# gregbugaj/marie-icr

Measured on AMD Instinct MI355X. Metric: pages/sec (2550x3300, ~40 lines/page), higher is better.
Workload: dtype f16; 1 GPU; BASELINE configs[2]: full detect->crop->recognize, 64 synthetic 2550x3300x3 u8 pages per GPU per step resident in HBM; DiT-base Mask R-CNN detector (resize to 1035x800, 1 pass, 8 pages per forward) + TrOCR-base recognizer on the generator's 40 ground-truth line boxes per page (fixed work), beam 3, 15+1 decoder steps; seeded random weights; f16 operands with fp32 accumulation is the 16-bit mode of ; crops_per_page=40

## Files before the change

include/marie_hip.h:

```cpp
#ifndef MARIE_HIP_H
#define MARIE_HIP_H

#include <stddef.h>
#include <stdint.h>

#ifdef __cplusplus
extern "C" {
#endif

#define MHIP_OK 0
#define MHIP_EINVAL (-22)
#define MHIP_ENOMEM (-12)
#define MHIP_EHIP (-5)
#define MHIP_ESTATE (-1)

#define MHIP_PREC_F16 0
#define MHIP_PREC_F32 1

typedef struct mhip_ctx mhip_ctx;
typedef struct mhip_crnn mhip_crnn;

int mhip_init(int device_id, mhip_ctx** out);
int mhip_destroy(mhip_ctx* ctx);
const char* mhip_last_error(mhip_ctx* ctx);
// ... 236 lines not shown
  int max_positions;
  int beam;
  int max_len_b;
  int min_len;
  int pad, eos;
  float embed_scale;
  int img_size;
} mhip_trocr_config;
int mhip_trocr_default_config(int model , mhip_trocr_config* cfg);
int mhip_trocr_max_len(const mhip_trocr_config* cfg);
int mhip_trocr_create(mhip_ctx* ctx, int precision, const mhip_trocr_config* cfg, mhip_trocr** out);
int mhip_trocr_destroy(mhip_trocr* m);
int mhip_trocr_set_tensor(mhip_trocr* m, const char* key, const float* data, const int64_t* shape, int ndim);
int mhip_trocr_finalize(mhip_trocr* m);
int mhip_trocr_alloc_arena(mhip_trocr* m);
int mhip_trocr_arena(mhip_trocr* m, int which , void** arena_dev, size_t* bytes);
size_t mhip_trocr_workspace_bytes(mhip_trocr* m, int n);
int mhip_trocr_set_decode_gate(mhip_trocr* m, mhip_gate* gate);
int mhip_trocr_generate(mhip_trocr* m, const uint8_t* crops_dev, int n, int swap_rb, int32_t* tokens_out,
                        int32_t* lengths_out, float* scores_out);
int mhip_trocr_generate_host(mhip_trocr* m, const uint8_t* crops_host, int n, int swap_rb, int32_t* tokens_out,
                             int32_t* lengths_out, float* scores_out, float* enc_tokens_out, float* step0_logits_out);
int mhip_trocr_encode_begin(mhip_trocr* m, int max_crops);
int mhip_trocr_encode_fragments(mhip_trocr* m, const uint8_t* base_dev, const mhip_crop_desc* descs_host, int n, int swap_rb);
int mhip_trocr_encoded(mhip_trocr* m);
int mhip_trocr_decode(mhip_trocr* m, int32_t* tokens_out, int32_t* lengths_out, float* scores_out);
int mhip_trocr_generate_fragments(mhip_trocr* m, const uint8_t* base_dev, const mhip_crop_desc* descs_host, int n,
                                  int swap_rb, int32_t* tokens_out, int32_t* lengths_out, float* scores_out);
int mhip_trocr_generate_trace_host(mhip_trocr* m, const uint8_t* crops_host, int n, int swap_rb, int32_t* tokens_out,
                                   int32_t* lengths_out, float* scores_out, float* trace_scores, int32_t* trace_tokens,
                                   int32_t* trace_beams, int* steps_out);
int mhip_cross_attention_host(mhip_ctx* ctx, const float* q, const float* enc, const float* wk, const float* wv,
                              const float* bv, int crops, int beam, int heads, int n_tok, int enc_dim, float* out);
int mhip_decode_attention_host(mhip_ctx* ctx, int precision, int heads, int n_keys, int nq, int rows, int slots, int kv_rows,
                               const float* q, const float* k, const float* v, const int32_t* anc, int anc_ld,
                               int force_generic, float* out);

typedef struct mhip_layoutlmv3 mhip_layoutlmv3;
typedef struct mhip_layoutlmv3_config {
  int hidden, layers, heads, ffn;
  int vocab, type_vocab;
  int max_position_embeddings;
  int max_2d_position_embeddings;
  int coordinate_size, shape_size;
  int input_size, patch;
  int rel_pos_bins, max_rel_pos;
  int rel_2d_pos_bins, max_rel_2d_pos;
  float layer_norm_eps;
  int pad_id;
  int num_labels;
  int max_text;
} mhip_layoutlmv3_config;
int mhip_layoutlmv3_default_config(mhip_layoutlmv3_config* cfg);
int mhip_layoutlmv3_create(mhip_ctx* ctx, int precision, const mhip_layoutlmv3_config* cfg, mhip_layoutlmv3** out);
int mhip_layoutlmv3_destroy(mhip_layoutlmv3* m);
int mhip_layoutlmv3_set_tensor(mhip_layoutlmv3* m, const char* key, const float* data, const int64_t* shape, int ndim);
int mhip_layoutlmv3_finalize(mhip_layoutlmv3* m);
int mhip_layoutlmv3_alloc_arena(mhip_layoutlmv3* m);
int mhip_layoutlmv3_arena(mhip_layoutlmv3* m, void** arena_dev, size_t* bytes);
int mhip_layoutlmv3_set_resample(mhip_layoutlmv3* m, int filter);
int mhip_layoutlmv3_seq_len(const mhip_layoutlmv3_config* cfg);
int mhip_layoutlmv3_bucket(int relative_position, int num_buckets, int max_distance);
int mhip_layoutlmv3_classify(mhip_layoutlmv3* m, const uint8_t* base_dev, const mhip_crop_desc* pages_host, int n,
                             const int32_t* ids, const int32_t* bbox, const int32_t* attention_mask, float* logits_out);
int mhip_layoutlmv3_hidden_host(mhip_layoutlmv3* m, const uint8_t* pages_host, size_t pages_bytes,
                                const mhip_crop_desc* pages_desc, int n, const int32_t* ids, const int32_t* bbox,
// ... 65 lines not shown
```

marie_icr_amd/_lib.py:

```python
from __future__ import annotations

import ctypes as C
import os
import weakref

import numpy as np

_HERE = os.path.dirname(os.path.abspath(__file__))
LIB_PATH = os.environ.get("MARIE_HIP_LIB") or os.path.join(_HERE, "libmarie_hip.so")

PREC_F16 = 0
PREC_F32 = 1

_vp, _i, _sz = C.c_void_p, C.c_int, C.c_size_t
_SIGNATURES = (
    ("mhip_init", _i, [_i, C.POINTER(_vp)]),
    ("mhip_destroy", _i, [_vp]),
    ("mhip_last_error", C.c_char_p, [_vp]),
    ("mhip_set_stream", _i, [_vp, _vp]),
    ("mhip_synchronize", _i, [_vp]),
    ("mhip_device_info", _i, [_vp, C.c_char_p, _sz, C.POINTER(_i), C.POINTER(_sz)]),
    ("mhip_memcpy_dev", _i, [_vp, _vp, _vp, _sz]),
    ("mhip_gate_create", _i, [_vp, C.POINTER(_vp)]),
    ("mhip_gate_destroy", _i, [_vp]),
# ... 64 lines not shown
    ("mhip_det_final_multi_host", _i, [_vp, _vp, _i, _vp, _i, _i, _i, _i, _i, _i, C.c_float, C.c_float, _i, _vp, _vp,
                                       _vp, _vp]),
    ("mhip_register_warp", _i, [_vp, _vp, _i, _i, C.c_size_t, _vp, _vp, _vp]),
    ("mhip_register_warp_host", _i, [_vp, _vp, _i, _i, _vp, _vp]),
    ("mhip_blackout_bboxes", _i, [_vp, _vp, _i, _i, _vp, _i, C.POINTER(_i)]),
    ("mhip_content_extents", _i, [_vp, _vp, _i, _i, _vp, _i, _i, _vp]),
    ("mhip_overlay_create", _i, [_vp, _i, _i, C.POINTER(_vp)]),
    ("mhip_overlay_destroy", _i, [_vp]),
    ("mhip_overlay_set_tensor", _i, [_vp, C.c_char_p, _vp, C.POINTER(C.c_int64), _i]),
    ("mhip_overlay_finalize", _i, [_vp]),
    ("mhip_overlay_padded_shape", _i, [_i, _i, C.POINTER(_i), C.POINTER(_i)]),
    ("mhip_overlay_forward", _i, [_vp, _vp, _i, _i, _vp]),
    ("mhip_overlay_forward_host", _i, [_vp, _vp, _i, _i, _vp, _vp]),
    ("mhip_overlay_blend", _i, [_vp, _vp, _vp, _vp, _sz]),
    ("mhip_trocr_default_config", _i, [_i, _vp]),
    ("mhip_trocr_max_len", _i, [_vp]),
    ("mhip_trocr_create", _i, [_vp, _i, _vp, C.POINTER(_vp)]),
    ("mhip_trocr_destroy", _i, [_vp]),
    ("mhip_trocr_set_tensor", _i, [_vp, C.c_char_p, _vp, C.POINTER(C.c_int64), _i]),
    ("mhip_trocr_finalize", _i, [_vp]),
    ("mhip_trocr_alloc_arena", _i, [_vp]),
    ("mhip_trocr_arena", _i, [_vp, _i, C.POINTER(_vp), C.POINTER(_sz)]),
    ("mhip_trocr_workspace_bytes", _sz, [_vp, _i]),
    ("mhip_trocr_set_decode_gate", _i, [_vp, _vp]),
    ("mhip_trocr_generate", _i, [_vp, _vp, _i, _i, _vp, _vp, _vp]),
    ("mhip_trocr_generate_host", _i, [_vp, _vp, _i, _i, _vp, _vp, _vp, _vp, _vp]),
    ("mhip_trocr_generate_fragments", _i, [_vp, _vp, _vp, _i, _i, _vp, _vp, _vp]),
    ("mhip_trocr_encode_begin", _i, [_vp, _i]),
    ("mhip_trocr_encode_fragments", _i, [_vp, _vp, _vp, _i, _i]),
    ("mhip_trocr_encoded", _i, [_vp]),
    ("mhip_trocr_decode", _i, [_vp, _vp, _vp, _vp]),
    ("mhip_trocr_generate_trace_host", _i, [_vp, _vp, _i, _i, _vp, _vp, _vp, _vp, _vp, _vp, C.POINTER(_i)]),
    ("mhip_cross_attention_host", _i, [_vp, _vp, _vp, _vp, _vp, _vp, _i, _i, _i, _i, _i, _vp]),
    ("mhip_decode_attention_host", _i, [_vp, _i, _i, _i, _i, _i, _i, _i, _vp, _vp, _vp, _vp, _i, _i, _vp]),
    ("mhip_gemm_ln_fold", _i, [_vp, _i, _vp]),
    ("mhip_ln_finalize", _i, [_vp, _vp, _i, _i, _vp, _vp, _i, _i, C.c_float]),
    ("mhip_token_init_split", _i, [_vp, _vp, _vp, _vp, _vp, _vp, _i, _i, _i, _i, _i]),
    ("mhip_layoutlmv3_default_config", _i, [_vp]),
    ("mhip_layoutlmv3_create", _i, [_vp, _i, _vp, C.POINTER(_vp)]),
    ("mhip_layoutlmv3_destroy", _i, [_vp]),
    ("mhip_layoutlmv3_set_tensor", _i, [_vp, C.c_char_p, _vp, C.POINTER(C.c_int64), _i]),
    ("mhip_layoutlmv3_finalize", _i, [_vp]),
    ("mhip_layoutlmv3_alloc_arena", _i, [_vp]),
    ("mhip_layoutlmv3_arena", _i, [_vp, C.POINTER(_vp), C.POINTER(_sz)]),
    ("mhip_layoutlmv3_set_resample", _i, [_vp, _i]),
    ("mhip_layoutlmv3_seq_len", _i, [_vp]),
    ("mhip_layoutlmv3_bucket", _i, [_i, _i, _i]),
    ("mhip_layoutlmv3_max_token_labels", _i, [_i]),
    ("mhip_layoutlmv3_classify", _i, [_vp, _vp, _vp, _i, _vp, _vp, _vp, _vp]),
    ("mhip_layoutlmv3_hidden_host", _i, [_vp, _vp, _sz, _vp, _i, _vp, _vp, _vp, _vp, _vp, _vp]),
    ("mhip_layoutlmv3_tag", _i, [_vp, _vp, _vp, _i, _vp, _i, _vp, _vp, _vp, _vp, _vp, _vp]),
    ("mhip_layoutlmv3_tag_host", _i, [_vp, _vp, _sz, _vp, _i, _vp, _i, _vp, _vp, _vp, _vp, _vp, _vp]),
    ("mhip_token_head_host", _i, [_vp, _i, _i, _i, _i, _vp, _vp, _vp, _vp, _vp, _vp, _vp, _vp]),
    ("mhip_attention_bias_host", _i, [_vp, _i, _i, _i, _vp, _vp, _vp, _vp, _vp, _vp, _vp, _vp, _vp, _vp, _i, _i, _i, _i, _vp]),
    ("mhip_vq_template_create", _i, [_vp, _vp, _i, _i, _i, _vp, _vp, _i, C.POINTER(_vp)]),
    ("mhip_vq_template_destroy", _i, [_vp]),
    ("mhip_vq_template_state", _i, [_vp, C.POINTER(_i), C.POINTER(_i), _vp, _vp]),
    ("mhip_vq_template_set_filters", _i, [_vp, _vp, _vp]),
    ("mhip_vq_match", _i, [_vp, _vp, _i, _i, _sz, _vp, _i, _i, _i, _vp, _i, _i, _vp]),
    ("mhip_vq_assign_host", _i, [_vp, _vp, _i, _i, _vp, _vp, _i, _vp]),
    ("mhip_vq_kmeans_step_host", _i, [_vp, _vp, _i, _i, _vp, _vp, _i, _vp, _vp, _vp, C.POINTER(C.c_double)]),
    ("mhip_vq_heatmap_host", _i, [_vp, _vp, _i, _i, _i, _vp, _vp, _vp, _vp]),
    ("mhip_vq_peaks_host", _i, [_vp, _vp, _i, _i, _i, _vp, _i, _vp]),
    ("mhip_clip_cosine_host", _i, [_vp, _vp, _vp, _i, _i, _i, _vp]),
    ("mhip_max_page_size", _i, [_i, _i, _i, _i, C.c_double, C.POINTER(_i), C.POINTER(_i)]),
    ("mhip_resize_area_u8", _i, [_vp, _vp, _i, _i, _i, C.c_size_t, _vp, _i, _i]),
# ... 296 lines not shown
```

marie_icr_amd/csrc/common.h:

```cpp
#pragma once
#include <hip/hip_runtime.h>
#include <stdint.h>
#include <stdio.h>
#include <string.h>

#include <mutex>
#include <string>
#include <vector>

#include "../../include/marie_hip.h"

enum MhipKernelId {
  MHIP_K_CONV_FIRST = 0,
  MHIP_K_CONV_IGEMM = 1,
  MHIP_K_LSTM_REC = 2,
  MHIP_K_CTC_DECODE = 3,
  MHIP_K_IMAGE_OPS = 4,
  MHIP_K_CCL = 5,
  MHIP_K_CROP_BATCH = 6,
  MHIP_K_ATTN = 7,
  MHIP_K_ATTN_FLASH = 8,
  MHIP_K_VIT_OPS = 9,
  MHIP_K_DET_OPS = 10,
  MHIP_K_DEC_OPS = 11,
// ... 299 lines not shown
int mhip_launch_subsample2(mhip_ctx* ctx, int precision, const void* in, void* out, int B, int H, int W, int C);

int mhip_launch_layernorm2(mhip_ctx* ctx, int precision, const float* x, const float* g, const float* b, float* y_f32,
                           void* y_t, int rows, int D, float eps);
int mhip_launch_embed_step(mhip_ctx* ctx, int precision, const int* tokens, const void* emb, const float* pos_row, float scale,
                           const float* g, const float* b, float* x, void* xt, int rows, int D, float eps);
constexpr int DEC_ATTN_MAX_KEYS = 640;
struct DecAttnDesc {
  const void* q = nullptr;
  const void* k = nullptr;
  const void* v = nullptr;
  void* out = nullptr;
  const int* anc = nullptr;
  int anc_ld = 0, slots = 0;
  int kv_rows = 0;
  int ldq = 0, ldk = 0, ldo = 0;
  int heads = 0, groups = 0, nq = 1, n_keys = 0;
  int force_generic = 0;
};
int mhip_launch_decode_attention(mhip_ctx* ctx, int precision, const DecAttnDesc& d);
struct CrossAbsorbDesc {
  const void* q = nullptr;
  int ldq = 0;
  const void* E = nullptr;
  int kv_rows = 0, n_keys = 0, enc_dim = 0;
  const void* wkt = nullptr;
  const void* wv = nullptr;
  const float* bv = nullptr;
  void* qt = nullptr;
  void* ct = nullptr;
  void* ao = nullptr;
  int ldo = 0;
  int crops = 0, beam = 1, heads = 0;
};
bool mhip_cross_absorb_supported(int enc_dim, int beam, int heads);
int mhip_launch_cross_absorbed(mhip_ctx* ctx, const CrossAbsorbDesc& d);
struct BeamCandDesc {
  const void* logits = nullptr;
  int logits_f16 = 0;
  int ld = 0, vocab = 0, beam = 1, bsz = 0;
  const float* cum = nullptr;
  int step = 0, max_len = 0, min_len = 1, pad = 1, eos = 2;
  float* cand_scores = nullptr;
  int* cand_tokens = nullptr;
  int* cand_beams = nullptr;
};
int mhip_launch_beam_candidates(mhip_ctx* ctx, const BeamCandDesc& d);
int mhip_launch_ancestry(mhip_ctx* ctx, const int* anc_old, int* anc_new, const int* parent, int rows, int ld, int step);
struct BeamState {
  int bsz = 0, beam = 1, max_len = 0, pad = 1, eos = 2;
  const float* cand_scores = nullptr;
  const int* cand_tokens = nullptr;
  const int* cand_beams = nullptr;
  int* tokens[2] = {nullptr, nullptr};
  int* last_tok = nullptr;
  int* parent = nullptr;
  float* cum = nullptr;
  unsigned char* ignore = nullptr;
  unsigned char* finished = nullptr;
  int* fin_count = nullptr;
  int* fin_tokens = nullptr;
  int* fin_len = nullptr;
  float* fin_score = nullptr;
  int* remaining = nullptr;
};
void mhip_beam_state_carve(Carver& ws, int bsz, int beam, int max_len, int pad, int eos, BeamState* st);
// ... 48 lines not shown
```

marie_icr_amd/csrc/cross_attn.hip:

```cpp
#include <math.h>

#include "common.h"

namespace {

typedef _Float16 half8v __attribute__((ext_vector_type(8)));
typedef _Float16 half4v __attribute__((ext_vector_type(4)));
typedef __fp16 fp16x4 __attribute__((__vector_size__(4 * sizeof(__fp16))));
typedef float float4v __attribute__((ext_vector_type(4)));

#ifndef CA_E_AUX
#define CA_E_AUX 2
#endif
__device__ __forceinline__ void glds16(const void* gsrc, void* lds_wave_base) {
  __builtin_amdgcn_global_load_lds((const __attribute__((address_space(1))) void*)gsrc,
                                   (__attribute__((address_space(3))) void*)lds_wave_base, 16, 0, CA_E_AUX);
}
__device__ __forceinline__ half4v lds_tr16(const char* p) {
  fp16x4 v = __builtin_amdgcn_ds_read_tr16_b64_v4f16((__attribute__((address_space(3))) fp16x4*)p);
  return __builtin_bit_cast(half4v, v);
}
__device__ __forceinline__ int swz(int row) { return ((row & 7) << 1) | ((row >> 3) & 1); }

template <int N>
__device__ __forceinline__ void wait_vm() {
  asm volatile("s_waitcnt vmcnt(%0)" ::"n"(N) : "memory");
}
template <int PER, int MAXT>
__device__ __forceinline__ void wait_vm_dyn(int tiles) {
  if constexpr (MAXT <= 0 || PER <= 0) {
    wait_vm<0>();
  } else {
    if (tiles >= MAXT) wait_vm<PER * MAXT>();
    else wait_vm_dyn<PER, MAXT - 1>(tiles);
  }
}

struct CrossArgs {
  const _Float16* E;
  const _Float16* qt;
  _Float16* ct;
  size_t crop_stride, tile_stride;
  int n_keys, heads;
};

#ifndef CA_TK
#define CA_TK 32
#endif
constexpr int TK = CA_TK;
static_assert(TK == 16 || TK == 32, "cross_attn key tile");
constexpr int RT = TK / 16;
constexpr int cross_slots(int ed, int w) {
  const int n = (160 * 1024 - 4 * w * 1024) / (TK * ed * 2);
  return n > 6 ? 6 : n;
}

template <int ED, int W, int NPW, int NI, bool FEED>
__device__ __forceinline__ void cross_tile(const char* __restrict__ sb, char* __restrict__ feed_dst, float4v* __restrict__ xb,
                                           const char* __restrict__ feed_src, const int (&dma_off)[NPW],
                                           const int (&a_off)[4], const int (&t_off)[8], const half8v (&qf)[ED / 64],
                                           float4v (&acc)[ED / 32], float& mref, float& lsum, int t, int n_keys, int wave, int lane) {
  constexpr int NW = 2 * W, ROWB = ED * 2, KS = ED / 64, MT = ED / 32;
  const int g = lane >> 4;
#ifdef CA_DMA_ONLY
    if (FEED) {
#pragma unroll
      for (int j = 0; j < NPW; ++j) {
        const int i = wave + j * NW;
        if (NI % NW == 0 || i < NI) glds16(feed_src + dma_off[j], feed_dst + i * 1024);
      }
    }
    if (CA_DMA_ONLY) __builtin_amdgcn_s_barrier();
    return;
#endif
    float4v s[2] = {(float4v){0.f, 0.f, 0.f, 0.f}, (float4v){0.f, 0.f, 0.f, 0.f}};
    constexpr int EVERY = (KS / NPW) > 0 ? (KS / NPW) : 1;
    constexpr int AHEAD = KS < 4 ? KS : 4;
    half8v a0[KS], a1[RT == 2 ? KS : 1];
#pragma unroll
    for (int ks = 0; ks < AHEAD; ++ks) {
      a0[ks] = *(const half8v*)(sb + a_off[ks & 3] + 256 * (ks >> 2));
      if (RT == 2) a1[ks] = *(const half8v*)(sb + a_off[ks & 3] + 256 * (ks >> 2) + 16 * ROWB);
    }
    __builtin_amdgcn_sched_barrier(0);
#pragma unroll
    for (int ks = 0; ks < KS; ++ks) {
      if (ks + AHEAD < KS) {
        a0[ks + AHEAD] = *(const half8v*)(sb + a_off[(ks + AHEAD) & 3] + 256 * ((ks + AHEAD) >> 2));
        if (RT == 2) a1[ks + AHEAD] = *(const half8v*)(sb + a_off[(ks + AHEAD) & 3] + 256 * ((ks + AHEAD) >> 2) + 16 * ROWB);
      }
      if (FEED && ks % EVERY == 0 && ks / EVERY < NPW) {
        const int j = ks / EVERY, i = wave + j * NW;
        if (NI % NW == 0 || i < NI) glds16(feed_src + dma_off[j], feed_dst + i * 1024);
      }
      __builtin_amdgcn_sched_barrier(0);
      s[0] = __builtin_amdgcn_mfma_f32_16x16x32_f16(a0[ks], qf[ks], s[0], 0, 0, 0);
      if (RT == 2) s[1] = __builtin_amdgcn_mfma_f32_16x16x32_f16(a1[RT == 2 ? ks : 0], qf[ks], s[1], 0, 0, 0);
      __builtin_amdgcn_sched_barrier(0);
    }
    if (FEED) {
#pragma unroll
      for (int j = (KS + EVERY - 1) / EVERY; j < NPW; ++j) {
        const int i = wave + j * NW;
        if (NI % NW == 0 || i < NI) glds16(feed_src + dma_off[j], feed_dst + i * 1024);
      }
    }
    xb[(wave * 2 + 0) * 64 + lane] = s[0];
    if (RT == 2) xb[(wave * 2 + 1) * 64 + lane] = s[1];
    __builtin_amdgcn_s_waitcnt(0xc07f);
    __builtin_amdgcn_s_barrier();
    s[0] += xb[((wave ^ 1) * 2 + 0) * 64 + lane];
    if (RT == 2) s[1] += xb[((wave ^ 1) * 2 + 1) * 64 + lane];
    const int key0 = t * TK;
    if (key0 + TK > n_keys) {
#pragma unroll
      for (int mt = 0; mt < RT; ++mt)
#pragma unroll
        for (int e = 0; e < 4; ++e)
          if (key0 + 16 * mt + 4 * g + e >= n_keys) s[mt][e] = -INFINITY;
    }
    float mx = fmaxf(fmaxf(s[0][0], s[0][1]), fmaxf(s[0][2], s[0][3]));
    if (RT == 2) mx = fmaxf(mx, fmaxf(fmaxf(s[1][0], s[1][1]), fmaxf(s[1][2], s[1][3])));
    mx = fmaxf(mx, __shfl_xor(mx, 16));
    mx = fmaxf(mx, __shfl_xor(mx, 32));
    if (t == 0) {
      mref = mx;
    } else if (__builtin_amdgcn_ballot_w64(mx > mref + 8.f) != 0) {
      const float nr = fmaxf(mref, mx), f = __builtin_amdgcn_exp2f(mref - nr);
      mref = nr;
      lsum *= f;
#pragma unroll
      for (int i = 0; i < MT; ++i) acc[i] *= f;
    }
    half8v pf = (half8v){0, 0, 0, 0, 0, 0, 0, 0};
#pragma unroll
    for (int mt = 0; mt < RT; ++mt)
#pragma unroll
      for (int e = 0; e < 4; ++e) {
// ... 12 lines not shown
    __builtin_amdgcn_sched_barrier(0);
#pragma unroll
    for (int mt = 0; mt < MT; ++mt) {
      if (mt + TAHEAD < MT) {
        tlo[mt + TAHEAD] = lds_tr16(sb + t_off[(mt + TAHEAD) & 7] + 256 * ((mt + TAHEAD) >> 3));
        if (RT == 2) thi[mt + TAHEAD] = lds_tr16(sb + t_off[(mt + TAHEAD) & 7] + 256 * ((mt + TAHEAD) >> 3) + 16 * ROWB);
      }
      __builtin_amdgcn_sched_barrier(0);
      if constexpr (RT == 2) {
        const half8v a = __builtin_shufflevector(tlo[mt], thi[mt], 0, 1, 2, 3, 4, 5, 6, 7);
        acc[mt] = __builtin_amdgcn_mfma_f32_16x16x32_f16(a, pf, acc[mt], 0, 0, 0);
      } else {
        acc[mt] = __builtin_amdgcn_mfma_f32_16x16x16f16(tlo[mt], pf4, acc[mt], 0, 0, 0);
      }
      __builtin_amdgcn_sched_barrier(0);
    }
}

template <int ED, int W>
__global__ __launch_bounds__(128 * W) void cross_attn_kernel(CrossArgs p) {
  extern __shared__ __attribute__((aligned(16))) char smem[];
  constexpr int NW = 2 * W;
  constexpr int ROWB = ED * 2;
  constexpr int HB = ED;
  constexpr int TILE_B = TK * ROWB;
  constexpr int NS = cross_slots(ED, W);
  constexpr int NI = TILE_B / 1024;
  constexpr int NPW = (NI + NW - 1) / NW;
  constexpr int KS = ED / 64, MT = ED / 32;
  const int tid = threadIdx.x, lane = tid & 63;
  const int wave = __builtin_amdgcn_readfirstlane(tid >> 6);
  const int beam = wave >> 1, hh = wave & 1;
  const int n = lane & 15, g = lane >> 4;
  const int crop = blockIdx.x;
  const char* Ec = (const char*)p.E + (size_t)crop * p.crop_stride;
  const int ntiles = (p.n_keys + TK - 1) / TK;
  float4v* xbuf = (float4v*)(smem + NS * TILE_B);

  int dma_off[NPW];
#pragma unroll
  for (int j = 0; j < NPW; ++j) {
    const int i = wave + j * NW;
    const int byte = i * 1024 + lane * 16;
    const int r = byte / ROWB, cp = (byte - r * ROWB) >> 4;
    const int c = (cp & ~15) | ((cp & 15) ^ swz(r));
    dma_off[j] = r * ROWB + c * 16;
  }
  auto issue = [&](int t, int slot) {
    const char* src = Ec + (size_t)t * p.tile_stride;
    char* dst = smem + slot * TILE_B;
#pragma unroll
    for (int j = 0; j < NPW; ++j) {
      const int i = wave + j * NW;
      if (NI % NW == 0 || i < NI) glds16(src + dma_off[j], dst + i * 1024);
    }
  };
  const bool short_wave = (NI % NW != 0) && (wave + (NPW - 1) * NW >= NI);

  half8v qf[KS];
  {
    const _Float16* qr = p.qt + ((size_t)(crop * W + beam) * 16 + n) * ED + hh * (ED / 2) + g * 8;
#pragma unroll
    for (int ks = 0; ks < KS; ++ks) {
      if (n < p.heads) qf[ks] = *(const half8v*)(qr + ks * 32);
      else qf[ks] = (half8v){0, 0, 0, 0, 0, 0, 0, 0};
    }
  }
  int a_off[4];
#pragma unroll
  for (int j = 0; j < 4; ++j) a_off[j] = n * ROWB + hh * HB + 16 * ((4 * j + g) ^ swz(n));
  int t_off[8];
  {
    const int q = n >> 2, pp = n & 3, row = 4 * g + q, x = swz(row);
#pragma unroll
    for (int j = 0; j < 8; ++j) t_off[j] = row * ROWB + hh * HB + 32 * (j ^ (x >> 1)) + 16 * ((pp >> 1) ^ (x & 1)) + 8 * (pp & 1);
  }

  float4v acc[MT];
#pragma unroll
  for (int i = 0; i < MT; ++i) acc[i] = (float4v){0.f, 0.f, 0.f, 0.f};
  float mref = 0.f, lsum = 0.f;

  constexpr int DEPTH = NS - 1;
  static_assert(NS >= 2 && DEPTH * NPW <= 60, "ring depth / vmcnt range");
#pragma unroll
  for (int i = 0; i < DEPTH; ++i)
    if (i < ntiles) issue(i, i);
  int slot = 0;
  const int nfeed = ntiles > DEPTH ? ntiles - DEPTH : 0;
  for (int t = 0; t < nfeed; ++t) {
    if (short_wave) wait_vm<(NPW - 1) * (DEPTH - 1)>();
    else wait_vm<NPW * (DEPTH - 1)>();
    __builtin_amdgcn_s_barrier();
    const char* feed_src = Ec + (size_t)(t + DEPTH) * p.tile_stride;
    char* feed_dst = smem + (slot == 0 ? NS - 1 : slot - 1) * TILE_B;
    cross_tile<ED, W, NPW, NI, true>(smem + slot * TILE_B, feed_dst, xbuf, feed_src, dma_off, a_off, t_off, qf, acc, mref, lsum, t,
                                     p.n_keys, wave, lane);
    slot = (slot == NS - 1) ? 0 : slot + 1;
  }
  for (int t = nfeed; t < ntiles; ++t) {
    const int after = min(DEPTH - 1, ntiles - 1 - t);
    if (short_wave) wait_vm_dyn<NPW - 1, DEPTH - 1>(after);
    else wait_vm_dyn<NPW, DEPTH - 1>(after);
    __builtin_amdgcn_s_barrier();
    cross_tile<ED, W, NPW, NI, false>(smem + slot * TILE_B, smem, xbuf, Ec, dma_off, a_off, t_off, qf, acc, mref, lsum, t, p.n_keys,
                                      wave, lane);
    slot = (slot == NS - 1) ? 0 : slot + 1;
  }
  lsum += __shfl_xor(lsum, 16);
  lsum += __shfl_xor(lsum, 32);
  const float inv = 1.f / lsum;
  if (n < p.heads) {
    _Float16* o = p.ct + ((size_t)(crop * W + beam) * 16 + n) * ED + hh * (ED / 2) + 4 * g;
#pragma unroll
    for (int mt = 0; mt < MT; ++mt) {
      half4v h;
#pragma unroll
      for (int e = 0; e < 4; ++e) h[e] = (_Float16)(acc[mt][e] * inv);
      *(half4v*)(o + 16 * mt) = h;
    }
  }
}

template <int ED>
__global__ __launch_bounds__(256) void absorb_q_kernel(const _Float16* __restrict__ q, int ldq, const _Float16* __restrict__ wkt,
                                                      _Float16* __restrict__ qt, int rows) {
  __shared__ __attribute__((aligned(16))) _Float16 stage[4][64][72];
  const int lane = threadIdx.x & 63, wave = threadIdx.x >> 6, n = lane & 15, g = lane >> 4;
  const int h = blockIdx.y, r0 = blockIdx.x * 64;
  half8v b[4][2];
#pragma unroll
  for (int nt = 0; nt < 4; ++nt)
#pragma unroll
    for (int ks = 0; ks < 2; ++ks) {
      const int r = r0 + nt * 16 + n;
      if (r < rows) b[nt][ks] = *(const half8v*)(q + (size_t)r * ldq + h * 64 + ks * 32 + g * 8);
      else b[nt][ks] = (half8v){0, 0, 0, 0, 0, 0, 0, 0};
    }
  constexpr int MTW = ED / 64;
  const _Float16* wrow = wkt + ((size_t)h * ED + wave * (ED / 4) + n) * 64 + g * 8;
#pragma unroll 1
  for (int mg = 0; mg < MTW / 4; ++mg) {
#pragma unroll
    for (int mi = 0; mi < 4; ++mi) {
      const int mt = mg * 4 + mi;
      const half8v a0 = *(const half8v*)(wrow + (size_t)mt * 16 * 64);
      const half8v a1 = *(const half8v*)(wrow + (size_t)mt * 16 * 64 + 32);
#pragma unroll
      for (int nt = 0; nt < 4; ++nt) {
        float4v c = {0.f, 0.f, 0.f, 0.f};
        c = __builtin_amdgcn_mfma_f32_16x16x32_f16(a0, b[nt][0], c, 0, 0, 0);
        c = __builtin_amdgcn_mfma_f32_16x16x32_f16(a1, b[nt][1], c, 0, 0, 0);
        half4v o;
// ... 36 lines not shown
    for (int mt = 0; mt < 4; ++mt) a[mt] = *(const half8v*)(arow + (size_t)mt * 16 * ED + ks * 32);
#pragma unroll
    for (int mt = 0; mt < 4; ++mt)
#pragma unroll
      for (int nt = 0; nt < 4; ++nt) c[mt][nt] = __builtin_amdgcn_mfma_f32_16x16x32_f16(a[mt], b[nt], c[mt][nt], 0, 0, 0);
  }
#pragma unroll
  for (int mt = 0; mt < 4; ++mt)
#pragma unroll
    for (int nt = 0; nt < 4; ++nt) part[wave][mt * 4 + nt][lane] = c[mt][nt];
  __syncthreads();
  const int r = r0 + wave * 16 + n;
#pragma unroll
  for (int mt = 0; mt < 4; ++mt) {
    float4v v = part[0][mt * 4 + wave][lane];
#pragma unroll
    for (int w = 1; w < 4; ++w) v += part[w][mt * 4 + wave][lane];
    const float4v bb = *(const float4v*)(bv + h * 64 + mt * 16 + 4 * g);
    half4v o;
#pragma unroll
    for (int e = 0; e < 4; ++e) o[e] = (_Float16)(v[e] + bb[e]);
    if (r < rows) *(half4v*)(ao + (size_t)r * ldo + h * 64 + mt * 16 + 4 * g) = o;
  }
}

template <int ED>
int launch_ed(mhip_ctx* ctx, const CrossAbsorbDesc& d) {
  const int rows = d.crops * d.beam;
  PROF_LAUNCH(ctx, MHIP_K_DEC_OPS, hipLaunchKernelGGL((absorb_q_kernel<ED>), dim3((rows + 63) / 64, d.heads), dim3(256), 0, ctx->stream,
                                                     (const _Float16*)d.q, d.ldq, (const _Float16*)d.wkt, (_Float16*)d.qt, rows));
  CrossArgs a;
  a.E = (const _Float16*)d.E; a.qt = (const _Float16*)d.qt; a.ct = (_Float16*)d.ct;
  constexpr int TILE_B = TK * ED * 2;
  a.n_keys = d.n_keys; a.heads = d.heads;
  a.crop_stride = (size_t)d.kv_rows * ED * 2; a.tile_stride = TILE_B;
  const size_t lds = (size_t)cross_slots(ED, d.beam) * TILE_B + (size_t)d.beam * 4096;
#define CROSS_LAUNCH(WV)                                                                                                       \
  do {                                                                                                                         \
    static std::once_flag attr;                                                                                                \
    std::call_once(attr, [&] {                                                                                                 \
      (void)hipFuncSetAttribute((const void*)cross_attn_kernel<ED, WV>, hipFuncAttributeMaxDynamicSharedMemorySize, (int)lds); \
    });                                                                                                                        \
    PROF_LAUNCH(ctx, MHIP_K_CROSS_ATTN,                                                                                        \
                hipLaunchKernelGGL((cross_attn_kernel<ED, WV>), dim3(d.crops), dim3(128 * WV), lds, ctx->stream, a));          \
  } while (0)
  switch (d.beam) {
    case 1: CROSS_LAUNCH(1); break;
    case 2: CROSS_LAUNCH(2); break;
    case 3: CROSS_LAUNCH(3); break;
    default: CROSS_LAUNCH(4); break;
  }
#undef CROSS_LAUNCH
  PROF_LAUNCH(ctx, MHIP_K_DEC_OPS, hipLaunchKernelGGL((absorb_v_kernel<ED>), dim3((rows + 63) / 64, d.heads), dim3(256), 0, ctx->stream,
                                                     (const _Float16*)d.ct, (const _Float16*)d.wv, d.bv, (_Float16*)d.ao, d.ldo, rows));
  hipError_t e = hipGetLastError();
  if (e != hipSuccess) return mhip_fail(ctx, MHIP_EHIP, "cross_attn launch: %s", hipGetErrorString(e));
  return 0;
}

}

bool mhip_cross_absorb_supported(int enc_dim, int beam, int heads) {
  return (enc_dim == 256 || enc_dim == 512 || enc_dim == 768 || enc_dim == 1024) && beam >= 1 && beam <= 4 && heads >= 1 && heads <= 16;
}

int mhip_launch_cross_absorbed(mhip_ctx* ctx, const CrossAbsorbDesc& d) {
  if (!d.q || !d.E || !d.wkt || !d.wv || !d.bv || !d.qt || !d.ct || !d.ao || d.crops < 1)
    return mhip_fail(ctx, MHIP_EINVAL, "cross_attn: null operand");
  if (!mhip_cross_absorb_supported(d.enc_dim, d.beam, d.heads) || d.n_keys < 1 || d.kv_rows < d.n_keys || d.ldq % 8 || d.ldo % 4)
    return mhip_fail(ctx, MHIP_EINVAL, "cross_attn: unsupported shape (enc_dim %d, beam %d, heads %d)", d.enc_dim, d.beam, d.heads);
  switch (d.enc_dim) {
    case 256: return launch_ed<256>(ctx, d);
    case 512: return launch_ed<512>(ctx, d);
    case 768: return launch_ed<768>(ctx, d);
    default: return launch_ed<1024>(ctx, d);
  }
}
// ... 1 lines not shown
```

marie_icr_amd/csrc/trocr_api.hip:

```cpp
#include <math.h>

#include "vit_internal.h"

struct mhip_trocr {
  mhip_ctx* ctx = nullptr;
  int precision = MHIP_PREC_F16;
  mhip_trocr_config cfg{};
  mhip_vit* vit = nullptr;
  TensorStore store;
  Arena arena;
  bool ready = false;
  uint8_t* frag_crops = nullptr;
  size_t frag_crops_bytes = 0;
  void* frag_scratch = nullptr;
  size_t frag_scratch_bytes = 0;
  bool absorb = false;
  mhip_gate* decode_gate = nullptr;
  int* h_remaining = nullptr;
  hipEvent_t rem_ev[2] = {nullptr, nullptr};
  char* enc_store = nullptr;
  int enc_cap = 0, enc_count = 0;
  size_t esz() const { return precision == MHIP_PREC_F16 ? 2 : 4; }
};

// ... 545 lines not shown
      MHIP_HIP(ctx, hipMalloc(&m->frag_scratch, scratch));
      m->frag_scratch_bytes = scratch;
    }
  }
  VitRun run;
  run.tokens_dst = m->enc_store + (size_t)m->enc_count * vg.npad * c.enc_dim * es;
  int rc = mhip_carve_workspace(ctx, [&](Carver& ws) { vit_carve(m->vit, ws, n, vg, &run); });
  if (rc) return rc;
  rc = mhip_pil_resize_fragments(ctx, base_dev, descs_host, n, m->frag_crops, S, S, MHIP_PIL_BICUBIC, m->frag_scratch, m->frag_scratch_bytes);
  if (rc) return rc;
  if ((rc = vit_encode(m->vit, m->frag_crops, n, S, S, S, S, swap_rb, &run))) return rc;
  m->enc_count += n;
  return MHIP_OK;
}

extern "C" int mhip_trocr_decode(mhip_trocr* m, int32_t* tokens_out, int32_t* lengths_out, float* scores_out) {
  if (!m || !tokens_out || !lengths_out || !scores_out) return MHIP_EINVAL;
  mhip_ctx* ctx = m->ctx;
  if (m->enc_count < 1) return mhip_fail(ctx, MHIP_EINVAL, "trocr: nothing encoded since mhip_trocr_encode_begin");
  MHIP_HIP(ctx, hipSetDevice(ctx->device));
  const int n = m->enc_count;
  VitGeom vg;
  vit_geometry(m->vit, m->cfg.img_size, m->cfg.img_size, &vg);
  TrocrDecodeBufs b;
  int rc = mhip_carve_workspace(ctx, [&](Carver& ws) { trocr_decode_carve(m, ws, n, vg, false, &b); });
  if (rc) return rc;
  MHIP_HIP(ctx, hipMemsetAsync(m->enc_store + (size_t)n * vg.npad * m->cfg.enc_dim * m->esz(), 0, (size_t)64 * m->cfg.enc_dim * m->esz(), ctx->stream));
  rc = trocr_decode(m, b, m->enc_store, vg, n, tokens_out, lengths_out, scores_out, nullptr, nullptr);
  m->enc_count = 0;
  return rc;
}


extern "C" int mhip_cross_attention_host(mhip_ctx* ctx, const float* q, const float* enc, const float* wk, const float* wv,
                                         const float* bv, int crops, int beam, int heads, int n_tok, int enc_dim, float* out) {
  if (!ctx || !q || !enc || !wk || !wv || !bv || !out || crops < 1 || n_tok < 1) return MHIP_EINVAL;
  if (!mhip_cross_absorb_supported(enc_dim, beam, heads)) return mhip_fail(ctx, MHIP_EINVAL, "cross_attention: unsupported shape");
  MHIP_HIP(ctx, hipSetDevice(ctx->device));
  const int D = heads * 64, M = crops * beam, npad = (n_tok + 7) / 8 * 8;
  const size_t rowsE = (size_t)crops * npad + 64;
  std::vector<_Float16> hq((size_t)M * D), hE(rowsE * enc_dim, (_Float16)0.f), hkt((size_t)D * enc_dim), hwv((size_t)D * enc_dim);
  for (size_t i = 0; i < hq.size(); ++i) hq[i] = (_Float16)q[i];
  for (int c = 0; c < crops; ++c)
    for (int s = 0; s < n_tok; ++s)
      for (int d = 0; d < enc_dim; ++d) hE[((size_t)c * npad + s) * enc_dim + d] = (_Float16)enc[((size_t)c * n_tok + s) * enc_dim + d];
  const float log2e = 1.4426950408889634f;
  for (int h = 0; h < heads; ++h)
    for (int d = 0; d < enc_dim; ++d)
      for (int j = 0; j < 64; ++j) hkt[((size_t)h * enc_dim + d) * 64 + j] = (_Float16)(wk[(size_t)(h * 64 + j) * enc_dim + d] * log2e);
  for (size_t i = 0; i < hwv.size(); ++i) hwv[i] = (_Float16)wv[i];
  const size_t scr = (size_t)M * 16 * enc_dim * 2;
  char *dq = nullptr, *dE = nullptr, *dkt = nullptr, *dwv = nullptr, *qt = nullptr, *ct = nullptr, *ao = nullptr;
  float* dbv = nullptr;
  int rc = mhip_carve_workspace(ctx, [&](Carver& ws) {
    dq = ws.take(hq.size() * 2); dE = ws.take(hE.size() * 2); dkt = ws.take(hkt.size() * 2);
    dwv = ws.take(hwv.size() * 2); dbv = ws.take<float>((size_t)D * 4);
    qt = ws.take(scr); ct = ws.take(scr); ao = ws.take((size_t)M * D * 2);
  });
  if (rc) return rc;
  MHIP_HIP(ctx, hipMemcpyAsync(dq, hq.data(), hq.size() * 2, hipMemcpyHostToDevice, ctx->stream));
  MHIP_HIP(ctx, hipMemcpyAsync(dE, hE.data(), hE.size() * 2, hipMemcpyHostToDevice, ctx->stream));
  MHIP_HIP(ctx, hipMemcpyAsync(dkt, hkt.data(), hkt.size() * 2, hipMemcpyHostToDevice, ctx->stream));
  MHIP_HIP(ctx, hipMemcpyAsync(dwv, hwv.data(), hwv.size() * 2, hipMemcpyHostToDevice, ctx->stream));
  MHIP_HIP(ctx, hipMemcpyAsync(dbv, bv, (size_t)D * 4, hipMemcpyHostToDevice, ctx->stream));
  CrossAbsorbDesc cd;
  cd.q = dq; cd.ldq = D; cd.E = dE; cd.kv_rows = npad; cd.n_keys = n_tok; cd.enc_dim = enc_dim;
  cd.wkt = dkt; cd.wv = dwv; cd.bv = dbv; cd.qt = qt; cd.ct = ct; cd.ao = ao; cd.ldo = D;
  cd.crops = crops; cd.beam = beam; cd.heads = heads;
  if ((rc = mhip_launch_cross_absorbed(ctx, cd))) return rc;
  std::vector<_Float16> ho((size_t)M * D);
  MHIP_HIP(ctx, hipMemcpyAsync(ho.data(), ao, ho.size() * 2, hipMemcpyDeviceToHost, ctx->stream));
  MHIP_HIP(ctx, hipStreamSynchronize(ctx->stream));
  for (size_t i = 0; i < ho.size(); ++i) out[i] = (float)ho[i];
  return MHIP_OK;
}

template <typename T>
static void to_elems(const float* src, size_t n, std::vector<char>& dst, size_t off, size_t count, size_t src_ld, size_t dst_ld) {
  T* d = (T*)dst.data();
  for (size_t i = 0; i < count; ++i)
    for (size_t j = 0; j < n; ++j) d[off + i * dst_ld + j] = (T)src[i * src_ld + j];
}

extern "C" int mhip_decode_attention_host(mhip_ctx* ctx, int precision, int heads, int n_keys, int nq, int rows, int slots,
                                          int kv_rows, const float* q, const float* k, const float* v, const int32_t* anc,
                                          int anc_ld, int force_generic, float* out) {
  if (!ctx || !q || !k || !v || !out) return MHIP_EINVAL;
  if (precision != MHIP_PREC_F16 && precision != MHIP_PREC_F32) return mhip_fail(ctx, MHIP_EINVAL, "unknown precision %d", precision);
  if (heads < 1 || heads > 16 || n_keys < 1 || nq < 1 || rows < 1 || rows % nq)
    return mhip_fail(ctx, MHIP_EINVAL, "decode_attention_host: heads %d n_keys %d nq %d rows %d", heads, n_keys, nq, rows);
  const bool self = anc != nullptr;
  if (self && (nq != 1 || slots < 1 || anc_ld < std::min(n_keys, DEC_ATTN_MAX_KEYS + 1)))
    return mhip_fail(ctx, MHIP_EINVAL, "decode_attention_host: self-attention needs nq 1, slots >= 1, anc_ld >= n_keys");
  if (!self && kv_rows < n_keys) return mhip_fail(ctx, MHIP_EINVAL, "decode_attention_host: kv_rows %d < n_keys %d", kv_rows, n_keys);
  const int hist = std::min(n_keys, DEC_ATTN_MAX_KEYS + 1);
  if (self)
    for (int r = 0; r < rows; ++r)
      for (int s = 0; s < hist; ++s)
        if (anc[(size_t)r * anc_ld + s] < 0 || anc[(size_t)r * anc_ld + s] >= slots)
          return mhip_fail(ctx, MHIP_EINVAL, "decode_attention_host: ancestry slot out of range at row %d step %d", r, s);
  MHIP_HIP(ctx, hipSetDevice(ctx->device));
  const int D = heads * 64, groups = rows / nq;
  const size_t es = precision == MHIP_PREC_F16 ? 2 : 4;
  const int ldq = self ? 3 * D : D, ldk = self ? 3 * D : D;
  const size_t nq_el = (size_t)rows * ldq;
  const size_t nk_el = self ? (size_t)hist * slots * ldk : (size_t)groups * kv_rows * D;
  std::vector<char> hq(nq_el * es), hk(nk_el * es), hv(self ? 0 : nk_el * es);
// ... 47 lines not shown
```

Before: 95.89 pages/s.

## Make cross-attention kernel persistent across crops with continuous tile prefetch

The cross-attention kernel now launches at most one block per CU, and each block loops over several crops. Its DMA ring keeps prefetching tiles straight from one crop into the next, and it also prefetches the next crop's query fragments, so the pipeline never drains between crops. The last tile of each crop fetches only the rows it needs instead of the padded tile, and the ring is zeroed when that path matters. Vmcnt is now tracked dynamically, which adds bookkeeping and branchy waitcnt selection. A test entry point exposes the grid cap and the padding value.

Result: no change. 95.69 pages/s (median of 2 runs) (-0.2%).

```diff
diff --git a/include/marie_hip.h b/include/marie_hip.h
--- a/include/marie_hip.h
+++ b/include/marie_hip.h
@@ -292,6 +292,9 @@
                                    int32_t* trace_beams, int* steps_out);
 int mhip_cross_attention_host(mhip_ctx* ctx, const float* q, const float* enc, const float* wk, const float* wv,
                               const float* bv, int crops, int beam, int heads, int n_tok, int enc_dim, float* out);
+int mhip_cross_attention_host_ex(mhip_ctx* ctx, const float* q, const float* enc, const float* wk, const float* wv,
+                                 const float* bv, int crops, int beam, int heads, int n_tok, int enc_dim, int grid_cap,
+                                 float pad_value, float* out);
 int mhip_decode_attention_host(mhip_ctx* ctx, int precision, int heads, int n_keys, int nq, int rows, int slots, int kv_rows,
                                const float* q, const float* k, const float* v, const int32_t* anc, int anc_ld,
                                int force_generic, float* out);
diff --git a/marie_icr_amd/_lib.py b/marie_icr_amd/_lib.py
--- a/marie_icr_amd/_lib.py
+++ b/marie_icr_amd/_lib.py
@@ -120,6 +120,7 @@
     ("mhip_trocr_decode", _i, [_vp, _vp, _vp, _vp]),
     ("mhip_trocr_generate_trace_host", _i, [_vp, _vp, _i, _i, _vp, _vp, _vp, _vp, _vp, _vp, C.POINTER(_i)]),
     ("mhip_cross_attention_host", _i, [_vp, _vp, _vp, _vp, _vp, _vp, _i, _i, _i, _i, _i, _vp]),
+    ("mhip_cross_attention_host_ex", _i, [_vp, _vp, _vp, _vp, _vp, _vp, _i, _i, _i, _i, _i, _i, C.c_float, _vp]),
     ("mhip_decode_attention_host", _i, [_vp, _i, _i, _i, _i, _i, _i, _i, _vp, _vp, _vp, _vp, _i, _i, _vp]),
     ("mhip_gemm_ln_fold", _i, [_vp, _i, _vp]),
     ("mhip_ln_finalize", _i, [_vp, _vp, _i, _i, _vp, _vp, _i, _i, C.c_float]),
diff --git a/marie_icr_amd/csrc/common.h b/marie_icr_amd/csrc/common.h
--- a/marie_icr_amd/csrc/common.h
+++ b/marie_icr_amd/csrc/common.h
@@ -355,6 +355,7 @@
   void* ao = nullptr;
   int ldo = 0;
   int crops = 0, beam = 1, heads = 0;
+  int grid_cap = 0;
 };
 bool mhip_cross_absorb_supported(int enc_dim, int beam, int heads);
 int mhip_launch_cross_absorbed(mhip_ctx* ctx, const CrossAbsorbDesc& d);
diff --git a/marie_icr_amd/csrc/cross_attn.hip b/marie_icr_amd/csrc/cross_attn.hip
--- a/marie_icr_amd/csrc/cross_attn.hip
+++ b/marie_icr_amd/csrc/cross_attn.hip
@@ -36,12 +36,39 @@
   }
 }
 
+template <int LO, int HI>
+__device__ __forceinline__ void wait_vm_range(int n) {
+  if constexpr (LO == HI) {
+    wait_vm<LO>();
+  } else {
+    constexpr int MID = (LO + HI + 1) / 2;
+    if (n >= MID) wait_vm_range<MID, HI>(n);
+    else wait_vm_range<LO, MID - 1>(n);
+  }
+}
+template <int OFF>
+__device__ __forceinline__ void load_q16(half8v& d, const _Float16* p) {
+  asm volatile("global_load_dwordx4 %0, %1, off offset:%2" : "=&v"(d) : "v"(p), "n"(OFF) : "memory");
+}
+template <int KS, int I = 0>
+__device__ __forceinline__ void load_q(half8v (&qf)[KS], const _Float16* p) {
+  if constexpr (I < KS) {
+    load_q16<I * 64>(qf[I], p);
+    load_q<KS, I + 1>(qf, p);
+  }
+}
+template <int KS>
+__device__ __forceinline__ void pin_q(half8v (&qf)[KS]) {
+#pragma unroll
+  for (int ks = 0; ks < KS; ++ks) asm volatile("" : "+v"(qf[ks]));
+}
+
 struct CrossArgs {
   const _Float16* E;
   const _Float16* qt;
   _Float16* ct;
   size_t crop_stride, tile_stride;
-  int n_keys, heads;
+  int n_keys, heads, crops;
 };
 
 #ifndef CA_TK
@@ -55,24 +82,35 @@
   return n > 6 ? 6 : n;
 }
 
-template <int ED, int W, int NPW, int NI, bool FEED>
+template <int ED, int W, int NPW, int NI, bool FULL>
 __device__ __forceinline__ void cross_tile(const char* __restrict__ sb, char* __restrict__ feed_dst, float4v* __restrict__ xb,
-                                           const char* __restrict__ feed_src, const int (&dma_off)[NPW],
-                                           const int (&a_off)[4], const int (&t_off)[8], const half8v (&qf)[ED / 64],
-                                           float4v (&acc)[ED / 32], float& mref, float& lsum, int t, int n_keys, int wave, int lane) {
+                                           const char* __restrict__ feed_src, const unsigned (&dma_off)[NPW],
+                                           const int (&a_off)[4], const int (&t_off)[8], half8v (&qf)[ED / 64],
+                                           float4v (&acc)[ED / 32], float& mref, float& lsum, int t, int n_keys, int wave, int lane,
+                                           int nf_pre, int nf_mid, const _Float16* qnext) {
   constexpr int NW = 2 * W, ROWB = ED * 2, KS = ED / 64, MT = ED / 32;
   const int g = lane >> 4;
+  auto burst = [&](int nf) {
+#pragma unroll
+    for (int j = 0; j < NPW; ++j)
+      if (j < nf) glds16(feed_src + dma_off[j], feed_dst + (wave + j * NW) * 1024);
+  };
 #ifdef CA_DMA_ONLY
-    if (FEED) {
+    if (FULL) {
 #pragma unroll
       for (int j = 0; j < NPW; ++j) {
         const int i = wave + j * NW;
         if (NI % NW == 0 || i < NI) glds16(feed_src + dma_off[j], feed_dst + i * 1024);
       }
+    } else {
+      if (nf_pre > 0) burst(nf_pre);
+      if (qnext) load_q<KS>(qf, qnext);
+      if (nf_mid > 0) burst(nf_mid);
     }
     if (CA_DMA_ONLY) __builtin_amdgcn_s_barrier();
     return;
 #endif
+    if (!FULL && nf_pre > 0) burst(nf_pre);
     float4v s[2] = {(float4v){0.f, 0.f, 0.f, 0.f}, (float4v){0.f, 0.f, 0.f, 0.f}};
     constexpr int EVERY = (KS / NPW) > 0 ? (KS / NPW) : 1;
     constexpr int AHEAD = KS < 4 ? KS : 4;
@@ -89,7 +127,7 @@
         a0[ks + AHEAD] = *(const half8v*)(sb + a_off[(ks + AHEAD) & 3] + 256 * ((ks + AHEAD) >> 2));
         if (RT == 2) a1[ks + AHEAD] = *(const half8v*)(sb + a_off[(ks + AHEAD) & 3] + 256 * ((ks + AHEAD) >> 2) + 16 * ROWB);
       }
-      if (FEED && ks % EVERY == 0 && ks / EVERY < NPW) {
+      if (FULL && ks % EVERY == 0 && ks / EVERY < NPW) {
         const int j = ks / EVERY, i = wave + j * NW;
         if (NI % NW == 0 || i < NI) glds16(feed_src + dma_off[j], feed_dst + i * 1024);
       }
@@ -98,12 +136,15 @@
       if (RT == 2) s[1] = __builtin_amdgcn_mfma_f32_16x16x32_f16(a1[RT == 2 ? ks : 0], qf[ks], s[1], 0, 0, 0);
       __builtin_amdgcn_sched_barrier(0);
     }
-    if (FEED) {
+    if (FULL) {
 #pragma unroll
       for (int j = (KS + EVERY - 1) / EVERY; j < NPW; ++j) {
         const int i = wave + j * NW;
         if (NI % NW == 0 || i < NI) glds16(feed_src + dma_off[j], feed_dst + i * 1024);
       }
+    } else {
+      if (qnext) load_q<KS>(qf, qnext);
+      if (nf_mid > 0) burst(nf_mid);
     }
     xb[(wave * 2 + 0) * 64 + lane] = s[0];
     if (RT == 2) xb[(wave * 2 + 1) * 64 + lane] = s[1];
@@ -182,12 +223,13 @@
   const int wave = __builtin_amdgcn_readfirstlane(tid >> 6);
   const int beam = wave >> 1, hh = wave & 1;
   const int n = lane & 15, g = lane >> 4;
-  const int crop = blockIdx.x;
-  const char* Ec = (const char*)p.E + (size_t)crop * p.crop_stride;
+  const int grid = gridDim.x, crop0 = blockIdx.x;
   const int ntiles = (p.n_keys + TK - 1) / TK;
+  const int ncrops = (p.crops - crop0 + grid - 1) / grid;
+  const int F = ncrops * ntiles;
   float4v* xbuf = (float4v*)(smem + NS * TILE_B);
 
-  int dma_off[NPW];
+  unsigned dma_off[NPW];
 #pragma unroll
   for (int j = 0; j < NPW; ++j) {
     const int i = wave + j * NW;
@@ -196,26 +238,18 @@
     const int c = (cp & ~15) | ((cp & 15) ^ swz(r));
     dma_off[j] = r * ROWB + c * 16;
   }
-  auto issue = [&](int t, int slot) {
-    const char* src = Ec + (size_t)t * p.tile_stride;
-    char* dst = smem + slot * TILE_B;
-#pragma unroll
-    for (int j = 0; j < NPW; ++j) {
-      const int i = wave + j * NW;
-      if (NI % NW == 0 || i < NI) glds16(src + dma_off[j], dst + i * 1024);
-    }
+#ifdef CA_FETCH_PAD
+  const int ni_last = NI;
+#else
+  const int ni_last = ((p.n_keys - (ntiles - 1) * TK) * ROWB + 1023) / 1024;
+#endif
+  const int cnt_full = (NI - wave + NW - 1) / NW;
+  const int cnt_last = ni_last > wave ? (ni_last - wave + NW - 1) / NW : 0;
+  auto crop_E = [&](int k) { return (const char*)p.E + (size_t)(crop0 + k * grid) * p.crop_stride; };
+  auto crop_q = [&](int k) {
+    return p.qt + ((size_t)((crop0 + k * grid) * W + beam) * 16 + (n < p.heads ? n : 0)) * ED + hh * (ED / 2) + g * 8;
   };
-  const bool short_wave = (NI % NW != 0) && (wave + (NPW - 1) * NW >= NI);
-
-  half8v qf[KS];
-  {
-    const _Float16* qr = p.qt + ((size_t)(crop * W + beam) * 16 + n) * ED + hh * (ED / 2) + g * 8;
-#pragma unroll
-    for (int ks = 0; ks < KS; ++ks) {
-      if (n < p.heads) qf[ks] = *(const half8v*)(qr + ks * 32);
-      else qf[ks] = (half8v){0, 0, 0, 0, 0, 0, 0, 0};
-    }
-  }
+
   int a_off[4];
 #pragma unroll
   for (int j = 0; j < 4; ++j) a_off[j] = n * ROWB + hh * HB + 16 * ((4 * j + g) ^ swz(n));
@@ -233,42 +267,97 @@
 
   constexpr int DEPTH = NS - 1;
   static_assert(NS >= 2 && DEPTH * NPW <= 60, "ring depth / vmcnt range");
-#pragma unroll
-  for (int i = 0; i < DEPTH; ++i)
-    if (i < ntiles) issue(i, i);
-  int slot = 0;
-  const int nfeed = ntiles > DEPTH ? ntiles - DEPTH : 0;
-  for (int t = 0; t < nfeed; ++t) {
-    if (short_wave) wait_vm<(NPW - 1) * (DEPTH - 1)>();
-    else wait_vm<NPW * (DEPTH - 1)>();
+
+  if (ntiles <= NS && ni_last < NI) {
+    for (int i = tid * 16; i < NS * TILE_B; i += 128 * W * 16) *(uint4*)(smem + i) = make_uint4(0u, 0u, 0u, 0u);
+    __builtin_amdgcn_s_waitcnt(0xc07f);
     __builtin_amdgcn_s_barrier();
-    const char* feed_src = Ec + (size_t)(t + DEPTH) * p.tile_stride;
-    char* feed_dst = smem + (slot == 0 ? NS - 1 : slot - 1) * TILE_B;
-    cross_tile<ED, W, NPW, NI, true>(smem + slot * TILE_B, feed_dst, xbuf, feed_src, dma_off, a_off, t_off, qf, acc, mref, lsum, t,
-                                     p.n_keys, wave, lane);
+  }
+
+  half8v qf[KS];
+  load_q<KS>(qf, crop_q(0));
+  int issued = KS, qmark = KS;
+  int fk = 0, ft = 0;
+  const char* fsrc = crop_E(0);
+  auto feed_next = [&] {
+    if (++ft == ntiles) { ft = 0; ++fk; fsrc = crop_E(fk); }
+    else fsrc += p.tile_stride;
+  };
+  int mark[DEPTH];
+#pragma unroll
+  for (int i = 0; i < DEPTH; ++i) {
+    if (i < F) {
+      const int nf = ft == ntiles - 1 ? cnt_last : cnt_full;
+#pragma unroll
+      for (int j = 0; j < NPW; ++j)
+        if (j < nf) glds16(fsrc + dma_off[j], smem + i * TILE_B + (wave + j * NW) * 1024);
+      issued += nf;
+      feed_next();
+    }
+    mark[i] = issued;
+  }
+  int slot = 0, f = 0;
+  auto top = [&](int t) {
+    int allowed = issued - mark[0];
+    if (t == 0) allowed = min(allowed, issued - qmark);
+    if (allowed == NPW * (DEPTH - 1)) wait_vm<NPW * (DEPTH - 1)>();
+    else if (allowed == (NPW - 1) * (DEPTH - 1)) wait_vm<(NPW - 1) * (DEPTH - 1)>();
+    else wait_vm_range<0, 63>(min(allowed, 63));
+    pin_q<KS>(qf);
+    if (t == 0 && n >= p.heads) {
+#pragma unroll
+      for (int ks = 0; ks < KS; ++ks) qf[ks] = (half8v){0, 0, 0, 0, 0, 0, 0, 0};
+    }
+    __builtin_amdgcn_s_barrier();
+  };
+  auto bottom = [&](int nf, bool feeds) {
+    issued += nf;
+#pragma unroll
+    for (int i = 0; i + 1 < DEPTH; ++i) mark[i] = mark[i + 1];
+    mark[DEPTH - 1] = issued;
+    if (feeds) feed_next();
     slot = (slot == NS - 1) ? 0 : slot + 1;
-  }
-  for (int t = nfeed; t < ntiles; ++t) {
-    const int after = min(DEPTH - 1, ntiles - 1 - t);
-    if (short_wave) wait_vm_dyn<NPW - 1, DEPTH - 1>(after);
-    else wait_vm_dyn<NPW, DEPTH - 1>(after);
-    __builtin_amdgcn_s_barrier();
-    cross_tile<ED, W, NPW, NI, false>(smem + slot * TILE_B, smem, xbuf, Ec, dma_off, a_off, t_off, qf, acc, mref, lsum, t, p.n_keys,
-                                      wave, lane);
-    slot = (slot == NS - 1) ? 0 : slot + 1;
-  }
-  lsum += __shfl_xor(lsum, 16);
-  lsum += __shfl_xor(lsum, 32);
-  const float inv = 1.f / lsum;
-  if (n < p.heads) {
-    _Float16* o = p.ct + ((size_t)(crop * W + beam) * 16 + n) * ED + hh * (ED / 2) + 4 * g;
-#pragma unroll
-    for (int mt = 0; mt < MT; ++mt) {
-      half4v h;
-#pragma unroll
-      for (int e = 0; e < 4; ++e) h[e] = (_Float16)(acc[mt][e] * inv);
-      *(half4v*)(o + 16 * mt) = h;
-    }
+    ++f;
+  };
+  const int nfull = ntiles - 1 - DEPTH;
+  for (int k = 0; k < ncrops; ++k) {
+    int t = 0;
+    for (; t < nfull; ++t) {
+      top(t);
+      cross_tile<ED, W, NPW, NI, true>(smem + slot * TILE_B, smem + (slot == 0 ? NS - 1 : slot - 1) * TILE_B, xbuf, fsrc, dma_off, a_off,
+                                       t_off, qf, acc, mref, lsum, t, p.n_keys, wave, lane, 0, 0, nullptr);
+      bottom(cnt_full, true);
+    }
+    for (; t < ntiles; ++t) {
+      top(t);
+      const bool feeds = f + DEPTH < F, last = t == ntiles - 1;
+      const int nf = !feeds ? 0 : ft == ntiles - 1 ? cnt_last : cnt_full;
+      const bool more = last && f + 1 < F;
+      cross_tile<ED, W, NPW, NI, false>(smem + slot * TILE_B, smem + (slot == 0 ? NS - 1 : slot - 1) * TILE_B, xbuf, fsrc, dma_off, a_off,
+                                        t_off, qf, acc, mref, lsum, t, p.n_keys, wave, lane, last ? 0 : nf, last ? nf : 0,
+                                        more ? crop_q(k + 1) : nullptr);
+      if (more) { issued += KS; qmark = issued; }
+      bottom(nf, feeds);
+    }
+#ifndef CA_DMA_ONLY
+    lsum += __shfl_xor(lsum, 16);
+    lsum += __shfl_xor(lsum, 32);
+    const float inv = 1.f / lsum;
+    if (n < p.heads) {
+      _Float16* o = p.ct + ((size_t)((crop0 + k * grid) * W + beam) * 16 + n) * ED + hh * (ED / 2) + 4 * g;
+#pragma unroll
+      for (int mt = 0; mt < MT; ++mt) {
+        half4v h;
+#pragma unroll
+        for (int e = 0; e < 4; ++e) h[e] = (_Float16)(acc[mt][e] * inv);
+        *(half4v*)(o + 16 * mt) = h;
+      }
+    }
+    issued += MT;
+#endif
+#pragma unroll
+    for (int i = 0; i < MT; ++i) acc[i] = (float4v){0.f, 0.f, 0.f, 0.f};
+    lsum = 0.f;
   }
 }
 
@@ -371,7 +460,20 @@
   CrossArgs a;
   a.E = (const _Float16*)d.E; a.qt = (const _Float16*)d.qt; a.ct = (_Float16*)d.ct;
   constexpr int TILE_B = TK * ED * 2;
-  a.n_keys = d.n_keys; a.heads = d.heads;
+  a.n_keys = d.n_keys; a.heads = d.heads; a.crops = d.crops;
+  int grid = d.grid_cap;
+  if (grid <= 0) {
+    static int cus[64];
+    const int dev = ctx->device >= 0 && ctx->device < 64 ? ctx->device : 0;
+    if (!cus[dev]) {
+      int v = 0;
+      if (hipDeviceGetAttribute(&v, hipDeviceAttributeMultiprocessorCount, ctx->device) != hipSuccess || v < 1)
+        return mhip_fail(ctx, MHIP_EHIP, "cross_attn: cannot query the CU count");
+      cus[dev] = v;
+    }
+    grid = cus[dev];
+  }
+  if (grid > d.crops) grid = d.crops;
   a.crop_stride = (size_t)d.kv_rows * ED * 2; a.tile_stride = TILE_B;
   const size_t lds = (size_t)cross_slots(ED, d.beam) * TILE_B + (size_t)d.beam * 4096;
 #define CROSS_LAUNCH(WV)                                                                                                       \
@@ -381,7 +483,7 @@
       (void)hipFuncSetAttribute((const void*)cross_attn_kernel<ED, WV>, hipFuncAttributeMaxDynamicSharedMemorySize, (int)lds); \
     });                                                                                                                        \
     PROF_LAUNCH(ctx, MHIP_K_CROSS_ATTN,                                                                                        \
-                hipLaunchKernelGGL((cross_attn_kernel<ED, WV>), dim3(d.crops), dim3(128 * WV), lds, ctx->stream, a));          \
+                hipLaunchKernelGGL((cross_attn_kernel<ED, WV>), dim3(grid), dim3(128 * WV), lds, ctx->stream, a));             \
   } while (0)
   switch (d.beam) {
     case 1: CROSS_LAUNCH(1); break;
diff --git a/marie_icr_amd/csrc/trocr_api.hip b/marie_icr_amd/csrc/trocr_api.hip
--- a/marie_icr_amd/csrc/trocr_api.hip
+++ b/marie_icr_amd/csrc/trocr_api.hip
@@ -601,14 +601,14 @@
 }
 
 
-extern "C" int mhip_cross_attention_host(mhip_ctx* ctx, const float* q, const float* enc, const float* wk, const float* wv,
-                                         const float* bv, int crops, int beam, int heads, int n_tok, int enc_dim, float* out) {
+static int cross_attention_host(mhip_ctx* ctx, const float* q, const float* enc, const float* wk, const float* wv, const float* bv,
+                                int crops, int beam, int heads, int n_tok, int enc_dim, int grid_cap, float pad_value, float* out) {
   if (!ctx || !q || !enc || !wk || !wv || !bv || !out || crops < 1 || n_tok < 1) return MHIP_EINVAL;
   if (!mhip_cross_absorb_supported(enc_dim, beam, heads)) return mhip_fail(ctx, MHIP_EINVAL, "cross_attention: unsupported shape");
   MHIP_HIP(ctx, hipSetDevice(ctx->device));
   const int D = heads * 64, M = crops * beam, npad = (n_tok + 7) / 8 * 8;
   const size_t rowsE = (size_t)crops * npad + 64;
-  std::vector<_Float16> hq((size_t)M * D), hE(rowsE * enc_dim, (_Float16)0.f), hkt((size_t)D * enc_dim), hwv((size_t)D * enc_dim);
+  std::vector<_Float16> hq((size_t)M * D), hE(rowsE * enc_dim, (_Float16)pad_value), hkt((size_t)D * enc_dim), hwv((size_t)D * enc_dim);
   for (size_t i = 0; i < hq.size(); ++i) hq[i] = (_Float16)q[i];
   for (int c = 0; c < crops; ++c)
     for (int s = 0; s < n_tok; ++s)
@@ -635,13 +635,26 @@
   CrossAbsorbDesc cd;
   cd.q = dq; cd.ldq = D; cd.E = dE; cd.kv_rows = npad; cd.n_keys = n_tok; cd.enc_dim = enc_dim;
   cd.wkt = dkt; cd.wv = dwv; cd.bv = dbv; cd.qt = qt; cd.ct = ct; cd.ao = ao; cd.ldo = D;
-  cd.crops = crops; cd.beam = beam; cd.heads = heads;
+  cd.crops = crops; cd.beam = beam; cd.heads = heads; cd.grid_cap = grid_cap;
   if ((rc = mhip_launch_cross_absorbed(ctx, cd))) return rc;
   std::vector<_Float16> ho((size_t)M * D);
   MHIP_HIP(ctx, hipMemcpyAsync(ho.data(), ao, ho.size() * 2, hipMemcpyDeviceToHost, ctx->stream));
   MHIP_HIP(ctx, hipStreamSynchronize(ctx->stream));
   for (size_t i = 0; i < ho.size(); ++i) out[i] = (float)ho[i];
   return MHIP_OK;
+}
+
+extern "C" int mhip_cross_attention_host(mhip_ctx* ctx, const float* q, const float* enc, const float* wk, const float* wv,
+                                         const float* bv, int crops, int beam, int heads, int n_tok, int enc_dim, float* out) {
+  return cross_attention_host(ctx, q, enc, wk, wv, bv, crops, beam, heads, n_tok, enc_dim, 0, 0.f, out);
+}
+
+extern "C" int mhip_cross_attention_host_ex(mhip_ctx* ctx, const float* q, const float* enc, const float* wk, const float* wv,
+                                            const float* bv, int crops, int beam, int heads, int n_tok, int enc_dim, int grid_cap,
+                                            float pad_value, float* out) {
+  if (grid_cap < 0 || !isfinite((float)(_Float16)pad_value))
+    return mhip_fail(ctx, MHIP_EINVAL, "cross_attention: grid_cap %d / pad_value %g (must be finite in f16)", grid_cap, pad_value);
+  return cross_attention_host(ctx, q, enc, wk, wv, bv, crops, beam, heads, n_tok, enc_dim, grid_cap, pad_value, out);
 }
 
 template <typename T>
```
